# anisanazim/Movie-Recommendation-Engine

Measured on AMD Instinct MI355X. Metric: item embeddings/sec + top-K ANN queries/sec, ML-25M d=256, 1/2/4/8 GPU, higher is better.
Workload: dtype f64 cdf / f32 features / fp4 sign planes (exact integer Hamming); 1 GPU; SYN-25M (ML-25M-shaped: U=162541 M=59047 R=25000095), F=128 H=256 d=256, 2 GCN layers, W=100 L=2 T=10, LSH 512-bit, 10000 queries K=11, rng=numpy (the reference's np.random MT19937 stream generated on device: neighbour ids bit-exact with the reference CPU path); global_items=59047, queries=10000, parallelism=item-shard x1

## Files before the change

### include/pinsage_hip.h

```cpp
#ifndef PINSAGE_HIP_H
#define PINSAGE_HIP_H

#include <stddef.h>
#include <stdint.h>

#ifdef __cplusplus
extern "C" {
#endif

#define PS_OK 0
#define PS_EINVAL (-1)
#define PS_ELAUNCH (-2)
#define PS_EWORKSPACE (-3)
#define PS_EUNSUPPORTED (-4)

#define PS_RNG_STREAM 0
#define PS_RNG_PHILOX 1
#define PS_RNG_STREAM_RAW 2

#define PS_RNG_STREAM_WALKS 3

#define PS_WALK_HALF_BUCKETS 0x100

typedef void *ps_stream_t;
// ... 85 lines not shown
                          ps_stream_t stream);

size_t ps_bn_stats_workspace_bytes(int64_t M, int N);
int ps_bn_batch_stats(const float *z, int64_t M, int N, const float *gamma, float eps, float momentum, float *running_mean,
                      float *running_var, float *mean, float *var, float *scale, void *workspace, size_t workspace_bytes,
                      ps_stream_t stream);
int ps_bn_apply(const float *z, int64_t M, int N, const float *mean, const float *scale, const float *beta, int flags, float *y,
                ps_stream_t stream);

#define PS_RELU 1
#define PS_L2NORM 2
#define PS_WPERM 4
int ps_permute_k(const float *W, int64_t rows, int K, int ld, float *out, ps_stream_t stream);
int ps_linear(const float *x, int64_t M, int K, const float *W, int ldw, const float *b, int N,
              const float *x2, int K2, const float *W2, int ldw2, int flags, float *y, ps_stream_t stream);

size_t ps_gcn_layer_workspace_bytes(int64_t M, int H);
int ps_gcn_layer(const float *x, int64_t M, int K, const float *W, int ldw, const float *b, int N, const float *h_full,
                 int64_t n_full, int H, const int32_t *ids, const int32_t *counts, const float *wts, const int32_t *nvalid,
                 int T, int64_t max_idx, int renorm, const float *W2, int ldw2, int flags, float *y, void *workspace,
                 size_t workspace_bytes, ps_stream_t stream);
int ps_gcn_order(const int32_t *ids, const int32_t *nvalid, int layers, int64_t M, int T, int64_t max_idx, int32_t *ord_out,
                 int32_t *tile_heavy_out, ps_stream_t stream);
int ps_gcn_layer_ordered(const float *x, int64_t M, int K, const float *W, int ldw, const float *b, int N, const float *h_full,
                         int64_t n_full, int H, const int32_t *ids, const int32_t *counts, const float *wts,
                         const int32_t *nvalid, int T, int64_t max_idx, int renorm, const float *W2, int ldw2, int flags, float *y,
                         void *workspace, size_t workspace_bytes, const int32_t *ord, const int32_t *tile_heavy,
                         ps_stream_t stream);

#define PS_LSH_STAGED 8
size_t ps_lsh_stage_bytes(int nbits, int D);
int ps_lsh_stage(const float *A, int nbits, int D, void *staged, size_t staged_bytes, ps_stream_t stream);
int ps_lsh_encode(const float *x, int64_t N, int D, const float *A, int nbits, uint8_t *codes, int flags, ps_stream_t stream);

size_t ps_hamming_topk_workspace_bytes(int64_t nq, int64_t N, int cs, int k);
int ps_hamming_topk(const uint8_t *qcodes, int64_t nq, const uint8_t *codes, int64_t N, int cs, int k,
                    int64_t id_offset, int32_t *dist, int64_t *ids,
                    void *workspace, size_t workspace_bytes, ps_stream_t stream);

size_t ps_lsh_planes_bytes(int64_t n, int cs);
int ps_lsh_expand(const uint8_t *codes, int64_t n, int cs, void *planes, ps_stream_t stream);
size_t ps_hamming_topk_mfma_workspace_bytes(int64_t nq, int64_t N, int cs, int k);
int ps_hamming_topk_mfma(const void *qplanes, int64_t nq, const void *dbplanes, int64_t N, int cs, int k,
                         int64_t id_offset, int32_t *dist, int64_t *ids,
                         void *workspace, size_t workspace_bytes, ps_stream_t stream);
int ps_hamming_topk_mfma_codes(const uint8_t *qcodes, int64_t nq, const void *dbplanes, int64_t N, int cs, int k,
                               int64_t id_offset, int32_t *dist, int64_t *ids,
                               void *workspace, size_t workspace_bytes, ps_stream_t stream);

int ps_topk_merge(const int32_t *dist_in, const int64_t *ids_in, int P, int64_t nq, int k,
                  int32_t *dist, int64_t *ids, ps_stream_t stream);
int ps_topk_merge_strided(const int32_t *dist_in, int64_t dist_stride, const int64_t *ids_in, int64_t ids_stride,
                          int P, int64_t nq, int k, int32_t *dist, int64_t *ids, ps_stream_t stream);

size_t ps_dot_topk_workspace_bytes(int64_t nq, int64_t N, int D, int k);
int ps_dot_topk(const float *E, int64_t N, int D, const int64_t *qidx, int64_t nq, int k, int exclude_self,
                float *vals, int64_t *ids, void *workspace, size_t workspace_bytes, ps_stream_t stream);

int ps_row_dot(const float *A, int64_t nA, const float *B, int64_t nB, int D, const int64_t *ia, const int64_t *ib, int64_t n,
               float *out, ps_stream_t stream);
int ps_rank_count(const float *E, int64_t N, int D, int64_t id_offset, const float *Q, int64_t nq, const float *thr,
                  const int64_t *tid, int64_t *count, ps_stream_t stream);

size_t ps_l2_topk_workspace_bytes(int64_t nq, int64_t N, int D, int k);
int ps_l2_topk(const float *X, int64_t N, int D, const float *Q, int64_t nq, int k, const int32_t *assign,
               const uint32_t *probe, int words, float *dist, int64_t *ids, void *workspace,
// ... 57 lines not shown
```

### movie-recommendation-engine_amd/csrc/hamming_mfma.hip

```cpp
#include "ps_select.h"
#include <type_traits>

namespace {

typedef int v4i __attribute__((ext_vector_type(4)));
typedef int v8i __attribute__((ext_vector_type(8)));
typedef float v16f __attribute__((ext_vector_type(16)));

#ifndef PS_HM_DEBUG
#define PS_HM_DEBUG 0
#endif
#if PS_HM_DEBUG & 32
__device__ unsigned long long ps_hm_counts[8];
#define PS_HM_COUNT(slot, n) do { if (MODE == 1 && lane == 0) atomicAdd(&ps_hm_counts[slot], (unsigned long long)(n)); } while (0)
extern "C" int ps_debug_hm_counts(unsigned long long *host, int reset) {
    unsigned long long z[8] = {};
    if (reset) return (int)hipMemcpyToSymbol(HIP_SYMBOL(ps_hm_counts), z, sizeof(z));
    return (int)hipMemcpyFromSymbol(host, HIP_SYMBOL(ps_hm_counts), sizeof(z));
}
#else
#define PS_HM_COUNT(slot, n) do {} while (0)
#endif
#if PS_HM_DEBUG & 512
__device__ unsigned long long ps_hm_times[4 * 4096];
extern "C" int ps_debug_hm_times_clear() {
    static unsigned long long z[4 * 4096];
    return (int)hipMemcpyToSymbol(HIP_SYMBOL(ps_hm_times), z, sizeof(z));
}
extern "C" int ps_debug_hm_times(unsigned long long *host) {
    return (int)hipMemcpyFromSymbol(host, HIP_SYMBOL(ps_hm_times), sizeof(unsigned long long) * 4 * 4096);
}
#endif
constexpr uint32_t EMPTY_KEY = PS_EMPTY32;
constexpr int NBUF = 4;
constexpr int WAVES = 8;
constexpr int PAD_TILES = 4;
constexpr float NO_DOT = -1048576.0f;
constexpr int entry_tiles(int KS) { return KS >= 4 ? 2 : 4; }
template <int KS> struct EntryTiles { static constexpr int value = entry_tiles(KS); };
template <int KS> struct EntryTiles2 { static constexpr int value = KS >= 8 ? 1 : KS == 4 ? 2 : 4; };
constexpr int ring_entries(bool db) { return db ? NBUF : 3; }
template <int KS, bool DB> constexpr int ring_bytes() {
    return ring_entries(DB) * (DB ? EntryTiles<KS>::value : EntryTiles2<KS>::value) * KS * 1024;
}
constexpr size_t column_bytes(int cap) { return (size_t)WAVES * cap * 64 * sizeof(uint32_t); }

__device__ __forceinline__ uint4 expand_word(uint32_t bits) {
    auto four = [](uint32_t n) { return (n | (n << 3) | (n << 6) | (n << 9)) & 0x1111u; };
    auto eight = [&](uint32_t byte) { return 0xaaaaaaaau ^ ((four(byte & 15u) | (four(byte >> 4) << 16)) << 3); };
    return make_uint4(eight(bits & 255u), eight((bits >> 8) & 255u), eight((bits >> 16) & 255u), eight(bits >> 24));
}

__global__ __launch_bounds__(256) void lsh_expand_kernel(const uint32_t *__restrict__ codes, int64_t n, int KS,
                                                         int64_t pieces, uint4 *__restrict__ planes) {
    for (int64_t p = (int64_t)blockIdx.x * blockDim.x + threadIdx.x; p < pieces; p += (int64_t)gridDim.x * blockDim.x) {
        const int lane = (int)(p & 63);
        const int64_t ts = p >> 6;
        const int s = (int)(ts % KS);
        const int64_t tile = ts / KS;
        const int64_t row = tile * 32 + (lane & 31);
        uint4 o = make_uint4(0u, 0u, 0u, 0u);
        if (row < n) o = expand_word(codes[row * (2 * KS) + 2 * s + (lane >> 5)]);
        planes[p] = o;
    }
}

struct HArgs {
    const unsigned char *qplanes;
    const uint32_t *qcodes;
    const unsigned char *dbplanes;
    int64_t nq, N;
    int64_t tile_begin, tile_end;
    int64_t tiles_per_slice;
    int nqb, slices;
    int k, nbits, shift;
    int cap;
    int64_t id_offset;
    const int32_t *thr0;
    int32_t *bl;
    int list_base;
    int32_t *out_d;
    int32_t *out_r;
};

// ... 946 lines not shown
```

### movie-recommendation-engine_amd/csrc/lsh_filter.hip

```cpp
#include "ps_common.h"

#ifndef PS_LSHF_DEBUG
#define PS_LSHF_DEBUG 0
#endif

#if PS_LSHF_DEBUG
__device__ float *ps_lshf_dump_buf;
extern "C" int ps_debug_lsh_dump(float *buf) { return (int)hipMemcpyToSymbol(HIP_SYMBOL(ps_lshf_dump_buf), &buf, sizeof buf); }
#endif

#if PS_LSHF_DEBUG == 2
#define LSHF_STAMP(slot) do { if (threadIdx.x == 0 && ps_lshf_dump_buf != nullptr) \
    reinterpret_cast<unsigned long long *>(ps_lshf_dump_buf)[(size_t)blockIdx.x * 16 + (slot)] = __builtin_readcyclecounter(); } while (0)
#define LSHF_NOW() __builtin_readcyclecounter()
#define LSHF_PUT(slot, v) do { if (threadIdx.x == 0 && ps_lshf_dump_buf != nullptr) \
    reinterpret_cast<unsigned long long *>(ps_lshf_dump_buf)[(size_t)blockIdx.x * 16 + (slot)] = (v); } while (0)
#else
#define LSHF_STAMP(slot) do {} while (0)
#define LSHF_NOW() 0ull
#define LSHF_PUT(slot, v) do {} while (0)
#endif

namespace {

typedef __bf16 bf16x8 __attribute__((ext_vector_type(8)));
typedef float f32x16 __attribute__((ext_vector_type(16)));
typedef float f32x4 __attribute__((ext_vector_type(4)));

constexpr uint32_t LSHF_MAGIC = 0x4653484cu;
constexpr int HEADER_BYTES = 64;
constexpr int LIST_CAP = 2048;
constexpr int MAX_NBITS = 1024;

// ... 34 lines not shown
#pragma unroll
        for (int e = 0; e < 8; ++e) {
            const float a = row[8 * (e >> 2) + (e & 3)];
            hi[e] = (__bf16)a;
            lo[e] = (__bf16)(a - (float)hi[e]);
        }
        bf16x8 *dst = reinterpret_cast<bf16x8 *>(img + off_slabs + (size_t)jt * slab_f4(KS) * 16);
        dst[(2 * s) * 64 + lane] = hi;
        dst[(2 * s + 1) * 64 + lane] = lo;
    }
    for (int64_t j = t0; j < nbits; j += step) {
        double ss = 0.0;
        for (int k = 0; k < D; ++k) {
            const double a = (double)A[(size_t)j * D + k];
            ss += a * a;
        }
        const double nrm = sqrt(ss);
        float na = __builtin_inff();
        if (nrm >= 0x1p-30 && nrm <= 0x1p30) na = (float)(nrm * (1.0 + 0x1p-10));
        float *dst = reinterpret_cast<float *>(img + off_slabs + ((size_t)(j / 32) * slab_f4(KS) + KS * 128) * 16);
        dst[j % 32] = na;
    }
}

struct FilterArgs {
    const float *x;
    int64_t N;
    const float *a32;
    const f32x4 *slabs;
    int nbits;
    uint32_t *codes;
    unsigned long long *counters;
    float c;
};

template <int KS, int JS>
__global__ __launch_bounds__(256, JS == 1 ? 2 : 1) void lsh_filter_kernel(const FilterArgs g) {
    constexpr int D = KS * 16, ROWS = 128 / JS, RG = 4 / JS, SF4 = slab_f4(KS), NQ = KS / 2;
    extern __shared__ f32x4 lds[];
    __shared__ uint32_t cnt, more;
    const int W = g.nbits / 32;
    f32x4 *slabL = lds;
    uint32_t *codesL = reinterpret_cast<uint32_t *>(lds + JS * SF4);
    uint32_t *flagsL = codesL + W * ROWS;
    uint32_t *listL = flagsL + W * ROWS;

    const int tid = threadIdx.x, lane = tid & 63, wave = tid >> 6;
    const int r = lane & 31, h = lane >> 5;
    const int rg = wave % RG, ph = wave / RG;
    const int64_t row0 = (int64_t)blockIdx.x * ROWS;
    const int64_t row = row0 + rg * 32 + r;
    const bool live = row < g.N;

    LSHF_STAMP(0);
    bf16x8 xh[KS], xl[KS];
    float ss = 0.f;
    {
        const float4 *xr = reinterpret_cast<const float4 *>(g.x + (live ? row : 0) * D);
#pragma unroll
        for (int s = 0; s < KS; ++s) {
#pragma unroll
            for (int t = 0; t < 2; ++t) {
                float4 v = xr[4 * s + 2 * t + h];
                if (!live) v = make_float4(0.f, 0.f, 0.f, 0.f);
                const float e[4] = {v.x, v.y, v.z, v.w};
#pragma unroll
                for (int q = 0; q < 4; ++q) {
                    const __bf16 hi = (__bf16)e[q];
                    xh[s][4 * t + q] = hi;
                    xl[s][4 * t + q] = (__bf16)(e[q] - (float)hi);
                    ss = fmaf(e[q], e[q], ss);
                }
            }
        }
    }
    ss += __shfl_xor(ss, 32);
    float thr = __builtin_inff();
    if (ss >= 0x1p-60f && ss <= 0x1p60f) thr = g.c * (sqrtf(ss) * (1.f + 0x1p-10f));

    const int iters = (W + JS - 1) / JS;
    f32x4 pre[JS][NQ], pna[JS];
#define LSHF_PREFETCH(it_)                                                             \
    _Pragma("unroll") for (int sl = 0; sl < JS; ++sl) {                                \
        const int jt_ = (it_) * JS + sl;                                                \
        if (jt_ < W) {                                                                  \
            const f32x4 *src = g.slabs + (size_t)jt_ * SF4;                            \
            _Pragma("unroll") for (int q = 0; q < NQ; ++q) pre[sl][q] = src[tid + 256 * q]; \
            if (tid < 8) pna[sl] = src[KS * 128 + tid];                                 \
        }                                                                               \
    }
    LSHF_PREFETCH(0)
    LSHF_STAMP(1);
    [[maybe_unused]] unsigned long long t_stage = 0ull, t_mfma = 0ull, t_epi = 0ull;
    for (int it = 0; it < iters; ++it) {
        const unsigned long long c0 = LSHF_NOW();
        __syncthreads();
#pragma unroll
        for (int sl = 0; sl < JS; ++sl) {
            if (it * JS + sl < W) {
#pragma unroll
                for (int q = 0; q < NQ; ++q) slabL[sl * SF4 + tid + 256 * q] = pre[sl][q];
                if (tid < 8) slabL[sl * SF4 + KS * 128 + tid] = pna[sl];
            }
        }
        __syncthreads();
        const unsigned long long c1 = LSHF_NOW();
        t_stage += c1 - c0;
        if (it + 1 < iters) { LSHF_PREFETCH(it + 1) }
        const int jt = it * JS + ph;
        if (jt < W) {
            const f32x4 *sb = slabL + ph * SF4;
            f32x16 acc, acc1;
#pragma unroll
            for (int e = 0; e < 16; ++e) acc[e] = acc1[e] = 0.f;
            f32x4 fh[3], fl[3];
            fh[0] = sb[lane];
            fl[0] = sb[64 + lane];
            if (KS > 1) {
                fh[1] = sb[2 * 64 + lane];
                fl[1] = sb[3 * 64 + lane];
            }
#pragma unroll
            for (int s = 0; s < KS; ++s) {
                if (s + 2 < KS) {
// ... 6 lines not shown
                    acc = __builtin_amdgcn_mfma_f32_32x32x16_bf16(al, xh[s], acc, 0, 0, 0);
                    acc1 = __builtin_amdgcn_mfma_f32_32x32x16_bf16(ah, xl[s], acc1, 0, 0, 0);
                    acc = __builtin_amdgcn_mfma_f32_32x32x16_bf16(ah, xh[s], acc, 0, 0, 0);
                } else {
                    acc1 = __builtin_amdgcn_mfma_f32_32x32x16_bf16(al, xh[s], acc1, 0, 0, 0);
                    acc = __builtin_amdgcn_mfma_f32_32x32x16_bf16(ah, xl[s], acc, 0, 0, 0);
                    acc1 = __builtin_amdgcn_mfma_f32_32x32x16_bf16(ah, xh[s], acc1, 0, 0, 0);
                }
                __builtin_amdgcn_sched_barrier(0);
            }
            acc += acc1;
            const unsigned long long c2 = LSHF_NOW();
            t_mfma += c2 - c1;
            uint32_t sm = 0u, fm = 0u;
#pragma unroll
            for (int gq = 0; gq < 4; ++gq) {
                const f32x4 na = sb[KS * 128 + 2 * gq + h];
#pragma unroll
                for (int q = 0; q < 4; ++q) {
                    const float f = acc[4 * gq + q];
#if PS_LSHF_DEBUG == 1
                    if (ps_lshf_dump_buf != nullptr && live) ps_lshf_dump_buf[row * g.nbits + jt * 32 + 8 * gq + 4 * h + q] = f;
#endif
                    const bool trusted = __builtin_fabsf(f) > thr * na[q];
                    sm |= (trusted && f >= 0.f ? 1u : 0u) << (8 * gq + q);
                    fm |= (trusted ? 0u : 1u) << (8 * gq + q);
                }
            }
            sm <<= 4 * h;
            fm <<= 4 * h;
            if (!live) fm = 0u;
            sm |= (uint32_t)__shfl_xor((int)sm, 32);
            fm |= (uint32_t)__shfl_xor((int)fm, 32);
            if (h == 0) {
                codesL[jt * ROWS + rg * 32 + r] = sm;
                flagsL[jt * ROWS + rg * 32 + r] = fm;
            }
            t_epi += LSHF_NOW() - c2;
        }
    }

#undef LSHF_PREFETCH
    LSHF_STAMP(2);
    LSHF_PUT(6, t_stage);
    LSHF_PUT(7, t_mfma);
    LSHF_PUT(8, t_epi);

    const int nwords = W * ROWS;
    unsigned long long nflag = 0ull;
    for (;;) {
        __syncthreads();
        if (tid == 0) {
            cnt = 0u;
            more = 0u;
        }
        __syncthreads();
        int mine = 0;
#pragma unroll 4
        for (int idx = tid; idx < nwords; idx += 256) mine += __builtin_popcount(flagsL[idx]);
        if (mine > 0) {
            uint32_t pos = atomicAdd(&cnt, (uint32_t)mine);
            if (pos + (uint32_t)mine > (uint32_t)LIST_CAP) more = 1u;
            for (int idx = tid; idx < nwords && pos < (uint32_t)LIST_CAP; idx += 256) {
                uint32_t m = flagsL[idx];
                if (m == 0u) continue;
                while (m != 0u && pos < (uint32_t)LIST_CAP) {
                    listL[pos++] = (uint32_t)idx * 32u + (uint32_t)__builtin_ctz(m);
                    m &= m - 1u;
                }
                flagsL[idx] = m;
            }
        }
        __syncthreads();
        LSHF_STAMP(3);
        const int n = cnt < (uint32_t)LIST_CAP ? (int)cnt : LIST_CAP;
        const bool again = more != 0u;
        for (int e = tid; e < n; e += 256) {
            const uint32_t ent = listL[e];
            const int idx = (int)(ent >> 5), b = (int)(ent & 31u);
            const int jt = idx / ROWS, rl = idx % ROWS;
            const float4 *xr = reinterpret_cast<const float4 *>(g.x + (row0 + rl) * D);
            const float4 *ar = reinterpret_cast<const float4 *>(g.a32 + (size_t)(jt * 32 + b) * D);
            float acc = 0.f;
#pragma unroll 16
            for (int k = 0; k < D / 4; ++k) {
                const float4 u = xr[k], v = ar[k];
                acc = fmaf(u.x, v.x, acc);
                acc = fmaf(u.y, v.y, acc);
                acc = fmaf(u.z, v.z, acc);
                acc = fmaf(u.w, v.w, acc);
            }
            if (acc >= 0.f) atomicOr(&codesL[idx], 1u << b);
        }
        nflag += (unsigned long long)n;
        if (!again) break;
    }
    __syncthreads();
    LSHF_STAMP(4);

    for (int i = tid; i < nwords; i += 256) {
        const int rl = i / W, w = i % W;
        if (row0 + rl < g.N) g.codes[(row0 + rl) * W + w] = codesL[w * ROWS + rl];
    }
    if (g.counters != nullptr && tid == 0) {
        const int64_t rows = g.N - row0 < ROWS ? g.N - row0 : ROWS;
        atomicAdd(g.counters, (unsigned long long)rows * (unsigned long long)g.nbits);
        atomicAdd(g.counters + 1, nflag);
    }
    LSHF_STAMP(5);
}

template <int KS, int JS>
size_t filter_lds(int nbits) {
    return (size_t)JS * slab_f4(KS) * 16 + (size_t)(nbits / 32) * (128 / JS) * 8 + (size_t)LIST_CAP * 4;
}

template <int KS, int JS>
int launch_filter(const FilterArgs &g, hipStream_t st) {
    const int64_t grid = ps_cdiv(g.N, 128 / JS);
    if (grid > 0x7fffffff) return PS_EUNSUPPORTED;
    const size_t lds = filter_lds<KS, JS>(g.nbits);
    hipLaunchKernelGGL((lsh_filter_kernel<KS, JS>), dim3((unsigned)grid), dim3(256), lds, st, g);
    PS_CHECK_LAUNCH();
    return PS_OK;
}

template <int KS, int JS>
bool allow_lds() {
    return ps_allow_lds(lsh_filter_kernel<KS, JS>, filter_lds<KS, JS>(MAX_NBITS));
}

}

extern "C" size_t ps_lsh_stage_bytes(int nbits, int D) { return served(nbits, D) ? stage_layout(nbits, D).total : 0; }

extern "C" int ps_lsh_stage(const float *A, int nbits, int D, void *staged, size_t staged_bytes, ps_stream_t stream) {
    if (nbits <= 0 || D <= 0 || !A || !staged) return PS_EINVAL;
    if (!served(nbits, D) || (reinterpret_cast<size_t>(A) | reinterpret_cast<size_t>(staged)) % 16 != 0) return PS_EUNSUPPORTED;
    const StageLayout l = stage_layout(nbits, D);
    if (staged_bytes < l.total) return PS_EINVAL;
    int64_t grid = ps_cdiv((int64_t)nbits * D, 256);
    if (grid > 1024) grid = 1024;
    hipLaunchKernelGGL(lsh_stage_kernel, dim3((unsigned)grid), dim3(256), 0, ps_stream(stream), A, nbits, D,
                       static_cast<unsigned char *>(staged), l.a32, l.slabs);
    PS_CHECK_LAUNCH();
    return PS_OK;
}

int psi_lsh_encode_staged(const float *x, int64_t N, int D, const void *staged, int nbits, uint8_t *codes, ps_stream_t stream) {
    if (!served(nbits, D) || (reinterpret_cast<size_t>(x) | reinterpret_cast<size_t>(staged)) % 16 != 0) return PS_EUNSUPPORTED;
    static PsPerDevice cus;
    int dv = 0;
    if (!ps_device_index(&dv)) return PS_ELAUNCH;
    int ncu = cus.get(dv);
    if (ncu == 0) {
        if (!(allow_lds<2, 1>() && allow_lds<4, 1>() && allow_lds<8, 1>() && allow_lds<16, 1>() && allow_lds<2, 2>() &&
              allow_lds<4, 2>() && allow_lds<8, 2>() && allow_lds<16, 2>()))
            return PS_ELAUNCH;
        if (hipDeviceGetAttribute(&ncu, hipDeviceAttributeMultiprocessorCount, dv) != hipSuccess || ncu <= 0) return PS_ELAUNCH;
        cus.set(dv, ncu);
    }
    const StageLayout l = stage_layout(nbits, D);
    const unsigned char *img = static_cast<const unsigned char *>(staged);
    const char *se = getenv("PS_LSH_STATS"), *re = getenv("PS_LSH_ROWS");
    FilterArgs g;
    g.x = x;
    g.N = N;
    g.a32 = reinterpret_cast<const float *>(img + l.a32);
    g.slabs = reinterpret_cast<const f32x4 *>(img + l.slabs);
    g.nbits = nbits;
    g.codes = reinterpret_cast<uint32_t *>(codes);
    g.counters = se && atoi(se) != 0 ? reinterpret_cast<unsigned long long *>(const_cast<unsigned char *>(img) + 16) : nullptr;
    g.c = 0x1p-12f * (D > 256 ? (float)D / 256.f : 1.f);
    const int rows = re ? atoi(re) : 0;
    const bool half = rows == 64 || (rows != 128 && ps_cdiv(N, 128) * 2 <= ncu);
    hipStream_t st = ps_stream(stream);
    switch (D / 16) {
        case 2: return half ? launch_filter<2, 2>(g, st) : launch_filter<2, 1>(g, st);
        case 4: return half ? launch_filter<4, 2>(g, st) : launch_filter<4, 1>(g, st);
        case 8: return half ? launch_filter<8, 2>(g, st) : launch_filter<8, 1>(g, st);
        default: return half ? launch_filter<16, 2>(g, st) : launch_filter<16, 1>(g, st);
    }
}
```

### movie-recommendation-engine_amd/pinsage_hip/dense.py

```python
from __future__ import annotations

import os

import torch

from . import native as nv


def _rowmajor(w):
    if w.dtype != torch.float32:
        raise TypeError("fp32 expected")
    if w.dim() != 2:
        raise ValueError("2-D matrix expected")
    if w.stride(1) != 1 or w.stride(0) < w.size(1):
        w = w.contiguous()
    return w, w.stride(0) if w.size(0) > 1 else max(w.stride(0), w.size(1))


def _require_cuda(*tensors):
    for t in tensors:
        if t is not None and not t.is_cuda:
            raise nv.NativeError("libpinsage_hip takes device (HBM) tensors; got a CPU tensor (no CPU fallback)")


# ... 186 lines not shown
    if max_idx is None:
        max_idx = n_full - 1
    if b is not None:
        b = b.contiguous()
    ids, nvalid = ids.contiguous(), nvalid.contiguous()
    counts = counts.contiguous() if counts is not None else None
    wts = wts.contiguous() if wts is not None else None
    flags = (nv.PS_RELU if relu else 0) | (nv.PS_L2NORM if l2norm else 0) | (nv.PS_WPERM if staged else 0)
    ws, wsb = nv.workspace("ps_gcn_layer_workspace_bytes", x.device, M, H)
    if wsb > 0:
        y = torch.empty((M, N), dtype=torch.float32, device=x.device)
        if order is not None:
            ord_, heavy = order
            if ord_.dtype != torch.int32 or heavy.dtype != torch.int32 or ord_.numel() != (M + 63) // 64 * 64 \
                    or heavy.numel() != (M + 63) // 64:
                raise ValueError("order: (int32[64 * ceil(M / 64)], int32[ceil(M / 64)]) of gcn_orders expected")
        with torch.cuda.device(x.device):
            if order is not None:
                rc = nv.lib().ps_gcn_layer_ordered(nv.ptr(x), M, K, nv.ptr(Wk, contiguous=False), ldw, nv.ptr(b), N, nv.ptr(h_full),
                                                   n_full, H, nv.ptr(ids), nv.ptr(counts), nv.ptr(wts), nv.ptr(nvalid), T, int(max_idx),
                                                   int(renorm), nv.ptr(W2k, contiguous=False), ldw2, flags, nv.ptr(y), nv.ptr(ws), wsb,
                                                   nv.ptr(ord_), nv.ptr(heavy), nv.stream())
            else:
                rc = nv.lib().ps_gcn_layer(nv.ptr(x), M, K, nv.ptr(Wk, contiguous=False), ldw, nv.ptr(b), N, nv.ptr(h_full), n_full, H,
                                           nv.ptr(ids), nv.ptr(counts), nv.ptr(wts), nv.ptr(nvalid), T, int(max_idx), int(renorm),
                                           nv.ptr(W2k, contiguous=False), ldw2, flags, nv.ptr(y), nv.ptr(ws), wsb, nv.stream())
        if rc != nv.PS_EUNSUPPORTED:
            nv.check(rc, "ps_gcn_layer")
            return y
    h_neigh = sampling.importance_pool(h_full, ids=ids, counts=counts, wts=wts, nvalid=nvalid, max_idx=max_idx, renorm=renorm)
    return linear(x, W, b, x2=h_neigh, W2=W2, relu=relu, l2norm=l2norm)


def lsh_encode(x, A):
    flags = nv.PS_LSH_STAGED if isinstance(A, StagedLsh) else nv.PS_WPERM if isinstance(A, StagedWeight) else 0
    if flags == nv.PS_LSH_STAGED:
        nbits, da, A = A.shape[0], A.shape[1], A.image
    elif flags:
        A = A.t
    _require_cuda(x, A)
    x = x.contiguous()
    A = A.contiguous()
    n, d = x.size(0), x.size(1)
    if flags != nv.PS_LSH_STAGED:
        nbits, da = A.size(0), A.size(1)
    if da != d:
        raise ValueError("projection matrix must be [nbits, dim]")
    codes = torch.empty((n, nbits // 8), dtype=torch.uint8, device=x.device)
    with torch.cuda.device(x.device):
        nv.call("ps_lsh_encode", nv.ptr(x), n, d, nv.ptr(A), nbits, nv.ptr(codes), flags, nv.stream())
    return codes


HAMMING_MAX_K = 64


def lsh_expand(codes):
    _require_cuda(codes)
    codes = codes.contiguous()
    n, cs = codes.size(0), codes.size(1)
    planes, nb = nv.workspace("ps_lsh_planes_bytes", codes.device, n, cs)
    if nb:
        with torch.cuda.device(codes.device):
            nv.call("ps_lsh_expand", nv.ptr(codes), n, cs, nv.ptr(planes), nv.stream())
    return planes


def hamming_mfma_supported(nq, N, cs, k):
    return nv.lib().ps_hamming_topk_mfma_workspace_bytes(nq, N, cs, k) > 0


def hamming_topk(qcodes, codes, k, id_offset=0, planes=None, use_mfma=True, out=None):
    _require_cuda(qcodes, codes)
    qcodes = qcodes.contiguous()
    codes = codes.contiguous()
    nq, cs = qcodes.size(0), qcodes.size(1)
    N = codes.size(0)
    if out is not None:
        dist, ids = out
        if (tuple(dist.shape) != (nq, k) or tuple(ids.shape) != (nq, k) or dist.dtype != torch.int32
                or ids.dtype != torch.int64 or not dist.is_contiguous() or not ids.is_contiguous()):
            raise ValueError("out must be contiguous (int32 [nq, k], int64 [nq, k])")
    if k > HAMMING_MAX_K or cs > 128 or (cs & (cs - 1)) != 0 or cs % 4 != 0:
        d, i = _hamming_topk_large_k(qcodes, codes, k, id_offset)
# ... 292 lines not shown
```

### movie-recommendation-engine_amd/pinsage_hip/native.py

```python
from __future__ import annotations

import ctypes as C
import os

import torch

_HERE = os.path.dirname(os.path.abspath(__file__))
SO_PATH = os.environ.get("PS_HIP_LIB") or os.path.join(_HERE, "libpinsage_hip.so")
_lib = None

PS_RNG_STREAM = 0
PS_RNG_PHILOX = 1
PS_RNG_STREAM_RAW = 2
PS_RNG_STREAM_WALKS = 3
PS_WALK_HALF_BUCKETS = 0x100
PS_RELU = 1
PS_L2NORM = 2
PS_WPERM = 4
PS_LSH_STAGED = 8
PS_HN_PER_QUERY, PS_HN_EXCLUDE_DIAG = 1, 2
PS_LOSS_SHARED, PS_LOSS_PER_QUERY, PS_LOSS_BATCH_HARD = 0, 1, 2
PS_PPR_NO_SKIP = 1
PS_OK, PS_EINVAL, PS_ELAUNCH, PS_EWORKSPACE, PS_EUNSUPPORTED = 0, -1, -2, -3, -4

# ... 22 lines not shown
    "ps_graph_stats": "i ppqqpp",
    "ps_walk_sample": "i pppqpqiiiippQIppppppppp",
    "ps_walk_sample_layers": "i pppqpqiiiippqQIpppppipppp",
    "ps_walk_paths": "i pppqpqiippQIipppp",
    "ps_uniform_offsets": "i pqpqiippp",
    "ps_mt19937_chunk_log2": "i",
    "ps_mt19937_window_shift": "i",
    "ps_mt19937_raw_stream": "i piqppppipipipipzp",
    "ps_mt19937_workspace_bytes": "z qq",
    "ps_mt19937_random_sample": "i piqqppppipipipzp",
    "ps_importance_pool": "i pqippppqiqipp",
    "ps_attention_weights": "i ppqipppqipp",
    "ps_gather_max": "i pqippqipp",
    "ps_pool_weights": "i ppppqiqiipp",
    "ps_gather_bwd_segment": "i",
    "ps_gather_bwd_workspace_bytes": "z qii",
    "ps_gather_bwd": "i ppqipppqippzp",
    "ps_gather_max_arg": "i pqippqippp",
    "ps_attention_bwd_rows_workspace_bytes": "z qi",
    "ps_attention_bwd_rows": "i pqippipppppqippppzp",
    "ps_attention_bwd_cols": "i ppqipppipqppzp",
    "ps_bn_stats_workspace_bytes": "z qi",
    "ps_bn_batch_stats": "i pqipffppppppzp",
    "ps_bn_apply": "i pqipppipp",
    "ps_permute_k": "i pqiipp",
    "ps_linear": "i pqipipipipiipp",
    "ps_gcn_layer_workspace_bytes": "z qi",
    "ps_gcn_layer": "i pqipipipqippppiqipiippzp",
    "ps_gcn_order": "i ppiqiqppp",
    "ps_gcn_layer_ordered": "i pqipipipqippppiqipiippzppp",
    "ps_lsh_stage_bytes": "z ii",
    "ps_lsh_stage": "i piipzp",
    "ps_lsh_encode": "i pqipipip",
    "ps_hamming_topk_workspace_bytes": "z qqii",
    "ps_hamming_topk": "i pqpqiiqpppzp",
    "ps_lsh_planes_bytes": "z qi",
    "ps_lsh_expand": "i pqipp",
    "ps_hamming_topk_mfma_workspace_bytes": "z qqii",
    "ps_hamming_topk_mfma": "i pqpqiiqpppzp",
    "ps_hamming_topk_mfma_codes": "i pqpqiiqpppzp",
    "ps_topk_merge": "i ppiqippp",
    "ps_topk_merge_strided": "i pqpqiqippp",
    "ps_dot_topk_workspace_bytes": "z qqii",
    "ps_dot_topk": "i pqipqiipppzp",
    "ps_row_dot": "i pqpqippqpp",
    "ps_rank_count": "i pqiqpqpppp",
    "ps_l2_topk_workspace_bytes": "z qqii",
    "ps_l2_topk": "i pqipqippipppzp",
    "ps_ivf_topk_workspace_bytes": "z qqiiiiq",
    "ps_ivf_topk": "i pqipiqppqpiipppzp",
    "ps_spmm_csr": "i ppppqiqqpp",
    "ps_cooc_planes_bytes": "z qqi",
    "ps_cooc_planes": "i pppqqqipzppp",
    "ps_cooc_pairs": "i pqqiqpqpqppp",
    "ps_cooc_pairs_sparse_workspace_bytes": "z qi",
    "ps_cooc_pairs_sparse": "i pppppppqqqqqipqpppzp",
    "ps_cooc_keys": "i pqqqppppppqpp",
    "ps_cooc_emit": "i ppqppp",
    "ps_hardest_negative": "i pqipqipppp",
    "ps_margin_loss": "i ppqipfppppp",
    "ps_margin_loss_bwd": "i pppqqiippppppp",
    "ps_ppr_shares": "i ppqpp",
    "ps_ppr_push_workspace_bytes": "z qq",
    "ps_ppr_push": "i pppqqppipqQiippzp",
    "ps_ppr_topk": "i pqqqqippppp",
}
# ... 23 lines not shown
    return _lib


def check(rc: int, what: str):
    if rc != 0:
        raise NativeError(f"{what}: {lib().ps_error_string(rc).decode()} (code {rc})")


class KernelTimer:

    def __init__(self):
        self.events = []

    def summary(self):
        torch.cuda.synchronize()
        out = {}
        for name, a, b in self.events:
            d = out.setdefault(name, {"launches": 0, "ms": 0.0})
            d["launches"] += 1
            d["ms"] += a.elapsed_time(b)
        for d in out.values():
            d["avg_ms"] = d["ms"] / d["launches"]
        return out


_timer = None


def set_timer(t):
    global _timer
    _timer = t


def call(name, *args):
    fn = getattr(lib(), name)
    if _timer is None:
        rc = fn(*args)
    else:
        a, b = torch.cuda.Event(enable_timing=True), torch.cuda.Event(enable_timing=True)
        a.record()
        rc = fn(*args)
        b.record()
        _timer.events.append((name, a, b))
    check(rc, name)


def ptr(t, contiguous=True):
    if t is None:
        return C.c_void_p(0)
    if not t.is_cuda:
        raise NativeError("libpinsage_hip takes device (HBM) pointers; got a CPU tensor")
    if contiguous and not t.is_contiguous():
        raise NativeError("tensor must be contiguous")
    return C.c_void_p(t.data_ptr())


def workspace(bytes_fn, device, *dims):
    nbytes = getattr(lib(), bytes_fn)(*dims)
    return (torch.empty(nbytes, dtype=torch.uint8, device=device) if nbytes else None), nbytes


_raw_stream = getattr(torch._C, "_cuda_getCurrentRawStream", None)
_get_device = getattr(torch._C, "_cuda_getDevice", None)


def stream():
    if _raw_stream is not None and _get_device is not None:
        return C.c_void_p(_raw_stream(_get_device()))
    return C.c_void_p(torch.cuda.current_stream().cuda_stream)


def require_gpu():
    if not torch.cuda.is_available():
        raise NativeError("the PinSage hot path needs an MI355X (torch.cuda is not available); "
                          "there is no CPU fallback")
    lib()
    return torch.device("cuda", torch.cuda.current_device())
# ... 7 lines not shown
```

### movie-recommendation-engine_amd/pinsage_hip/shard.py

```python
from __future__ import annotations

import os

import torch
import torch.distributed as dist

from . import dense, sampling


def shard_range(M, rank, world):
    chunk = (M + world - 1) // world
    lo = min(rank * chunk, M)
    return lo, min(lo + chunk, M), chunk


def _backend(group):
    return dist.get_backend(group) if dist.is_initialized() else None


class _Gather:

    def __init__(self, out, work=None, dev=None):
        self.out, self.work, self.dev = out, work, dev

# ... 72 lines not shown

class HipOps:

    def sample(self, sampler, nodes, T, shard=None):
        if shard is not None and getattr(sampler, "rng", None) == "numpy":
            M, lo = shard
            all_nodes = torch.arange(M, dtype=torch.int64, device=nodes.device)
            return sampler.sample_batch(nodes, T, stream_nodes=(all_nodes, lo))
        return sampler.sample_batch(nodes, T)

    def sample_layers(self, sampler, lo, hi, T, layers, shard=None):
        stream = None
        if shard is not None and getattr(sampler, "rng", None) == "numpy":
            stream = (range(shard[0]), shard[1])
        return sampler.sample_batches(range(lo, hi), T, layers, stream_nodes=stream, defer_state=True)

    def finish(self):
        dense.finish_rng_state()

    def pool(self, h_full, batch, max_idx):
        return sampling.importance_pool(h_full, batch, max_idx=max_idx)

    def linear(self, x, W, b, x2=None, W2=None, relu=False, l2norm=False):
        return dense.linear(x, W, b, x2=x2, W2=W2, relu=relu, l2norm=l2norm)

    def gcn_layer(self, x, W, b, h_full, batch, max_idx, W2, order=None):
        return dense.gcn_layer(x, W, b, h_full, batch.ids, batch.counts, batch.nvalid, W2, max_idx=max_idx, order=order)

    def gcn_orders(self, batches, max_idx):
        return dense.gcn_orders([b.ids for b in batches], [b.nvalid for b in batches], max_idx)

    def lsh_encode(self, x, A):
        return dense.lsh_encode(x, A)

    def stage_weight(self, W):
        return dense.stage_weight(W)

    def stage_lsh(self, A):
        return dense.stage_lsh(A)

    def lsh_planes(self, codes):
        return dense.lsh_expand(codes)

    def hamming_topk(self, q, codes, k, id_offset, planes=None, out=None):
        return dense.hamming_topk(q, codes, k, id_offset=id_offset, planes=planes, out=out)

    def topk_merge(self, d, i):
        return dense.topk_merge(d, i)

    def topk_merge_records(self, records, nq, k):
        return dense.topk_merge_records(records, nq, k)


class ShardedPinSage:

    def __init__(self, params, num_layers, sampler, num_items, ops=None, group=None, standin=None):
        self.P = params
        self.num_layers = num_layers
        self.sampler = sampler
        self.M = int(num_items)
        self.ops = ops if ops is not None else HipOps()
        self.group = group
        self.comm = Comm(group, standin=standin)
        self.rank, self.world = self.comm.rank, self.comm.world
        self.lo, self.hi, self.chunk = shard_range(self.M, self.rank, self.world)
        self._nodes = {}
# ... 98 lines not shown
            Wu = P[f"convs.{i}.lin_update.weight"]
            if self.fuse_self:
                W1, b1 = self._fused_layer(i, H)
                a_in = h
            else:
                a_in = ops.linear(h, P[f"convs.{i}.lin_self.weight"], P[f"convs.{i}.lin_self.bias"])
                W1, b1 = Wu[:, :H], P[f"convs.{i}.lin_update.bias"]
            h_full = pending.wait()
            if side is not None:
                torch.cuda.current_stream(dev).wait_event(ready[i])
            if self.fuse_self and hasattr(ops, "gcn_layer"):
                kw = {} if orders is None else {"order": orders[i]}
                h = ops.gcn_layer(a_in, self._w(("l1", i), W1), b1, h_full, batches[i], self.M - 1, self._w(("l2", i), Wu[:, H:]), **kw)
            else:
                h_neigh = ops.pool(h_full, batches[i], self.M - 1)
                h = ops.linear(a_in, self._w(("l1", i), W1), b1, x2=h_neigh, W2=self._w(("l2", i), Wu[:, H:]), relu=True, l2norm=True)
            if i + 1 < self.num_layers:
                pending = self.comm.gather_rows_async(h, self.chunk, "h")
        return ops.linear(h, self._w("out", P["output_proj.weight"]), P["output_proj.bias"], l2norm=True)

    def _staged_A(self, A):
        stage = getattr(self.ops, "stage_lsh", None) or getattr(self.ops, "stage_weight", None)
        if stage is None or not isinstance(A, torch.Tensor):
            return A
        ent = self._staged.get("A")
        if ent is None or ent[0] is not A or ent[1] != A._version:
            ent = self._staged["A"] = (A, A._version, stage(A))
        return ent[2]

    REPLICATE_CODES_BYTES = 64 << 20

    def build_index(self, emb_local, A):
        self.A = A
        self.codes = self.ops.lsh_encode(emb_local, self._staged_A(A))
        self.codes_all = None
        if self.world > 1 and self.M * int(self.codes.size(1)) <= self.REPLICATE_CODES_BYTES:
            self.codes_all = self.comm.gather_rows(self.codes, self.chunk, "codes")[: self.M]
        scanned = self.codes_all if self.codes_all is not None else self.codes
        self.planes = self.ops.lsh_planes(scanned) if hasattr(self.ops, "lsh_planes") else None
        return self.codes

    def search(self, q_local, k):
        ops = self.ops
        qc = ops.lsh_encode(q_local, self._staged_A(self.A))
        nq_local = qc.size(0)
        planes = getattr(self, "planes", None)
        if self.world > 1 and getattr(self, "codes_all", None) is not None:
            n = nq_local * k
            rec = (12 * n + 15) // 16 * 16
            mine = self.comm._buf("res", "mine", (1, rec), torch.uint8, qc.device, zero=True)
            ids_v = mine[0, : 8 * n].view(torch.int64).view(nq_local, k)
            dist_v = mine[0, 8 * n: 12 * n].view(torch.int32).view(nq_local, k)
            try:
                ops.hamming_topk(qc, self.codes_all, k, 0, planes=planes, out=(dist_v, ids_v))
            except TypeError:
                d, i = ops.hamming_topk(qc, self.codes_all, k, 0)
                dist_v.copy_(d)
                ids_v.copy_(i)
            allr = self.comm.gather_rows(mine, 1, "res")
            P_ = self.world
            return (allr[:, 8 * n: 12 * n].view(torch.int32).reshape(P_ * nq_local, k),
                    allr[:, : 8 * n].view(torch.int64).reshape(P_ * nq_local, k))
        qc_all = self.comm.gather_rows(qc, nq_local, "qcodes")
        if self.world == 1:
            return (ops.hamming_topk(qc_all, self.codes, k, self.lo, planes=planes) if planes is not None
                    else ops.hamming_topk(qc_all, self.codes, k, self.lo))
# ... 19 lines not shown
```

### movie-recommendation-engine_amd/utils/nearest_neighbors.py

```python
from __future__ import annotations

import time

import numpy as np
import torch

from pinsage_hip import dense
from pinsage_hip import native as nv

_INT_MAX_F = np.float32(2147483647)


def _faiss_float_randn(n, seed):
    def raw_stream(sd):
        bg = np.random.MT19937()
        bg._legacy_seeding(int(sd) & 0xFFFFFFFF)
        return bg
    g0 = raw_stream(seed)
    a0, b0 = (int(v) & 0x7FFFFFFF for v in g0.random_raw(2))
    nblock = 1 if n < 1024 else 1024
    out = np.empty(n, dtype=np.float32)
    inv = 1.0 / 4294967295.0
    for j in range(nblock):
        lo, hi = j * n // nblock, (j + 1) * n // nblock
# ... 64 lines not shown
        self.planes = None
        self.use_mfma = True
        self.device = nv.require_gpu()
        if self.rotate_data:
            A = lsh_rotation_matrix(self.d, self.nbits, seed=5, recipe=recipe)
        else:
            if self.d < self.nbits:
                raise ValueError("d >= nbits is required without rotate_data")
            A = np.eye(self.nbits, self.d, dtype=np.float32)
        self._set_A(A)

    def _set_A(self, A):
        A = torch.as_tensor(A, dtype=torch.float32)
        words = 1
        while words * 32 < A.size(0) and words < 32:
            words *= 2
        if words * 32 < A.size(0):
            words = (int(A.size(0)) + 31) // 32
        pad = words * 32 - A.size(0)
        if pad:
            A = torch.cat([A, torch.zeros((pad, A.size(1)), dtype=torch.float32)], dim=0)
        self.A = A.to(self.device).contiguous()
        self._staged = None

    def _staged_A(self):
        ent = self._staged
        if ent is None or ent[0] is not self.A or ent[1] != self.A._version:
            ent = self._staged = (self.A, self.A._version, dense.stage_lsh(self.A))
        return ent[2]

    def train(self, x):
        return None

    def _encode(self, x):
        x = torch.as_tensor(x, dtype=torch.float32).to(self.device)
        if x.dim() != 2 or x.size(1) != self.d:
            raise AssertionError(f"expected [n, {self.d}] vectors")
        return dense.lsh_encode(x, self._staged_A())

    def add(self, x):
        c = self._encode(x)
        self.codes = c if self.codes is None else torch.cat([self.codes, c], dim=0)
        self.ntotal = int(self.codes.size(0))
        self.planes = dense.lsh_expand(self.codes) if int(self.codes.size(1)) in (8, 16, 32, 64) else None

    def reset(self):
        self.codes, self.planes, self.ntotal = None, None, 0

    def search_device(self, x, k, id_offset=0):
        q = self._encode(x)
        codes = self.codes if self.codes is not None else torch.empty((0, self.code_size), dtype=torch.uint8,
                                                                       device=self.device)
        return dense.hamming_topk(q, codes, int(k), id_offset=id_offset, planes=self.planes, use_mfma=self.use_mfma)

    def search(self, x, k):
        dist, ids = self.search_device(x, k)
        d = dist.cpu().numpy().astype(np.float32)
        i = ids.cpu().numpy()
        d[i < 0] = _INT_MAX_F
        return d, i


class LSHIndex:

    rotation_recipe = "numpy"

    def __init__(self, dim, num_bits=256, num_tables=16):
        self.dim = dim
        self.num_bits = num_bits
        self.num_tables = num_tables
        self.index = _DeviceLSH(dim, num_bits, num_tables, recipe=self.rotation_recipe)

    def set_rotation(self, A):
        A = torch.as_tensor(A, dtype=torch.float32)
        if tuple(A.shape) != (self.num_bits, self.dim):
            raise ValueError("rotation must be [num_bits, dim]")
        self.index._set_A(A)
# ... 238 lines not shown
```

Measured before the change: 47.52 million items/s.

## Fuse LSH plane expansion into filter kernel and restructure flagged-bit refinement

The LSH filter kernel now writes the expanded fp4 sign planes directly from its LDS codes, so the separate lsh_expand pass is skipped when building the index. The flagged-word list is also built during the MFMA loop through per-wave segments, which removes the first full popcount scan. For JS==1 the exact dot-product refinement becomes a cooperative LDS-staged, prefetched computation in place of one thread per entry streaming rows. The cost is more LDS, more register pressure and extra complexity, plus a fallback path that expands separately when the fused path is unsupported.

```diff
diff --git a/include/pinsage_hip.h b/include/pinsage_hip.h
--- a/include/pinsage_hip.h
+++ b/include/pinsage_hip.h
@@ -141,6 +141,8 @@
 size_t ps_lsh_stage_bytes(int nbits, int D);
 int ps_lsh_stage(const float *A, int nbits, int D, void *staged, size_t staged_bytes, ps_stream_t stream);
 int ps_lsh_encode(const float *x, int64_t N, int D, const float *A, int nbits, uint8_t *codes, int flags, ps_stream_t stream);
+int ps_lsh_encode_planes(const float *x, int64_t N, int D, const void *staged, int nbits, uint8_t *codes, void *planes,
+                         ps_stream_t stream);
 
 size_t ps_hamming_topk_workspace_bytes(int64_t nq, int64_t N, int cs, int k);
 int ps_hamming_topk(const uint8_t *qcodes, int64_t nq, const uint8_t *codes, int64_t N, int cs, int k,
diff --git a/movie-recommendation-engine_amd/csrc/hamming_mfma.hip b/movie-recommendation-engine_amd/csrc/hamming_mfma.hip
--- a/movie-recommendation-engine_amd/csrc/hamming_mfma.hip
+++ b/movie-recommendation-engine_amd/csrc/hamming_mfma.hip
@@ -1,4 +1,5 @@
 #include "ps_select.h"
+#include "lsh_planes.h"
 #include <type_traits>
 
 namespace {
@@ -44,12 +45,6 @@
     return ring_entries(DB) * (DB ? EntryTiles<KS>::value : EntryTiles2<KS>::value) * KS * 1024;
 }
 constexpr size_t column_bytes(int cap) { return (size_t)WAVES * cap * 64 * sizeof(uint32_t); }
-
-__device__ __forceinline__ uint4 expand_word(uint32_t bits) {
-    auto four = [](uint32_t n) { return (n | (n << 3) | (n << 6) | (n << 9)) & 0x1111u; };
-    auto eight = [&](uint32_t byte) { return 0xaaaaaaaau ^ ((four(byte & 15u) | (four(byte >> 4) << 16)) << 3); };
-    return make_uint4(eight(bits & 255u), eight((bits >> 8) & 255u), eight((bits >> 16) & 255u), eight(bits >> 24));
-}
 
 __global__ __launch_bounds__(256) void lsh_expand_kernel(const uint32_t *__restrict__ codes, int64_t n, int KS,
                                                          int64_t pieces, uint4 *__restrict__ planes) {
diff --git a/movie-recommendation-engine_amd/csrc/lsh_filter.hip b/movie-recommendation-engine_amd/csrc/lsh_filter.hip
--- a/movie-recommendation-engine_amd/csrc/lsh_filter.hip
+++ b/movie-recommendation-engine_amd/csrc/lsh_filter.hip
@@ -1,4 +1,5 @@
 #include "ps_common.h"
+#include "lsh_planes.h"
 
 #ifndef PS_LSHF_DEBUG
 #define PS_LSHF_DEBUG 0
@@ -99,18 +100,27 @@
     uint32_t *codes;
     unsigned long long *counters;
     float c;
+    uint4 *planes;
+    int64_t plane_pieces;
 };
+
+__host__ __device__ constexpr int area_f4(int KS, int JS) {
+    return JS == 1 && slab_f4(KS) < 2048 ? 2048 : JS * slab_f4(KS);
+}
 
 template <int KS, int JS>
 __global__ __launch_bounds__(256, JS == 1 ? 2 : 1) void lsh_filter_kernel(const FilterArgs g) {
     constexpr int D = KS * 16, ROWS = 128 / JS, RG = 4 / JS, SF4 = slab_f4(KS), NQ = KS / 2;
+    constexpr int PF = KS >= 16 ? 4 : 2;
     extern __shared__ f32x4 lds[];
-    __shared__ uint32_t cnt, more;
+    constexpr int SEG = LIST_CAP / 4;
+    __shared__ uint32_t cnt, more, segn[4];
     const int W = g.nbits / 32;
     f32x4 *slabL = lds;
-    uint32_t *codesL = reinterpret_cast<uint32_t *>(lds + JS * SF4);
+    uint32_t *codesL = reinterpret_cast<uint32_t *>(lds + area_f4(KS, JS));
     uint32_t *flagsL = codesL + W * ROWS;
     uint32_t *listL = flagsL + W * ROWS;
+    uint16_t *wordL = reinterpret_cast<uint16_t *>(listL + LIST_CAP);
 
     const int tid = threadIdx.x, lane = tid & 63, wave = tid >> 6;
     const int r = lane & 31, h = lane >> 5;
@@ -157,6 +167,11 @@
         }                                                                               \
     }
     LSHF_PREFETCH(0)
+    if (tid == 0) {
+        cnt = 0u;
+        more = 0u;
+    }
+    int wcnt = 0;
     LSHF_STAMP(1);
     [[maybe_unused]] unsigned long long t_stage = 0ull, t_mfma = 0ull, t_epi = 0ull;
     for (int it = 0; it < iters; ++it) {
@@ -229,6 +244,14 @@
             if (!live) fm = 0u;
             sm |= (uint32_t)__shfl_xor((int)sm, 32);
             fm |= (uint32_t)__shfl_xor((int)fm, 32);
+            const bool fw = h == 0 && fm != 0u;
+            const unsigned long long wm = __ballot(fw);
+            if (fw) {
+                const int at = wcnt + (int)__builtin_amdgcn_mbcnt_lo((uint32_t)wm, 0u);
+                if (at < SEG) wordL[wave * SEG + at] = (uint16_t)(jt * ROWS + rg * 32 + r);
+                else more = 1u;
+            }
+            wcnt += __builtin_popcountll(wm);
             if (h == 0) {
                 codesL[jt * ROWS + rg * 32 + r] = sm;
                 flagsL[jt * ROWS + rg * 32 + r] = fm;
@@ -238,26 +261,125 @@
     }
 
 #undef LSHF_PREFETCH
+    if (lane == 0) segn[wave] = (uint32_t)(wcnt < SEG ? wcnt : SEG);
     LSHF_STAMP(2);
     LSHF_PUT(6, t_stage);
     LSHF_PUT(7, t_mfma);
     LSHF_PUT(8, t_epi);
 
     const int nwords = W * ROWS;
+    const f32x4 *xb = reinterpret_cast<const f32x4 *>(g.x + row0 * D), *ab = reinterpret_cast<const f32x4 *>(g.a32);
+    f32x4 *pieceL = lds;
     unsigned long long nflag = 0ull;
+    __syncthreads();
+    const int s1 = (int)segn[0], s2 = s1 + (int)segn[1], s3 = s2 + (int)segn[2];
+    const int nw = s3 + (int)segn[3];
+    for (int e = tid; e < nw; e += 256) {
+        const int w = (e >= s1 ? 1 : 0) + (e >= s2 ? 1 : 0) + (e >= s3 ? 1 : 0);
+        const uint32_t idx = wordL[w * SEG + e - (w == 3 ? s3 : w == 2 ? s2 : w == 1 ? s1 : 0)];
+        uint32_t m = flagsL[idx];
+        listL[e] = idx * 32u + (uint32_t)__builtin_ctz(m);
+        m &= m - 1u;
+        if (m != 0u) {
+            uint32_t pos = (uint32_t)nw + atomicAdd(&cnt, (uint32_t)__builtin_popcount(m));
+            while (m != 0u && pos < (uint32_t)LIST_CAP) {
+                listL[pos++] = idx * 32u + (uint32_t)__builtin_ctz(m);
+                m &= m - 1u;
+            }
+            if (m != 0u) more = 1u;
+        }
+        flagsL[idx] = m;
+    }
+    __syncthreads();
+    int n = (uint32_t)nw + cnt < (uint32_t)LIST_CAP ? nw + (int)cnt : LIST_CAP;
+    bool again = more != 0u;
+    LSHF_STAMP(3);
     for (;;) {
+        if constexpr (JS == 2) {
+            for (int e = tid; e < n; e += 256) {
+                const uint32_t ent = listL[e];
+                const int idx = (int)(ent >> 5), b = (int)(ent & 31u);
+                const f32x4 *xr = xb + (idx % ROWS) * (D / 4), *ar = ab + ((idx / ROWS) * 32 + b) * (D / 4);
+                float acc = 0.f;
+#pragma unroll 16
+                for (int k = 0; k < D / 4; ++k) {
+                    const f32x4 u = xr[k], v = ar[k];
+                    acc = fmaf(u[0], v[0], acc);
+                    acc = fmaf(u[1], v[1], acc);
+                    acc = fmaf(u[2], v[2], acc);
+                    acc = fmaf(u[3], v[3], acc);
+                }
+                if (acc >= 0.f) atomicOr(&codesL[idx], 1u << b);
+            }
+        }
+        for (int base = 0; JS == 1 && base < n; base += 256) {
+            const int m = n - base < 256 ? n - base : 256;
+            const int q = tid & 3, sw = (tid >> 4) & 3;
+            int xo[4], ao[4];
+#pragma unroll
+            for (int i = 0; i < 4; ++i) {
+                const int el = 64 * i + (tid >> 2);
+                const uint32_t ent = listL[base + (el < m ? el : 0)];
+                const int idx = (int)(ent >> 5), b = (int)(ent & 31u);
+                xo[i] = (idx % ROWS) * (D / 4) + q;
+                ao[i] = ((idx / ROWS) * 32 + b) * (D / 4) + q;
+            }
+            const uint32_t mine = listL[base + (tid < m ? tid : 0)];
+            f32x4 px[PF][4], pa[PF][4];
+#pragma unroll
+            for (int p = 0; p < PF; ++p) {
+#pragma unroll
+                for (int i = 0; i < 4; ++i) {
+                    px[p][i] = xb[xo[i] + 4 * p];
+                    pa[p][i] = ab[ao[i] + 4 * p];
+                }
+            }
+            float acc = 0.f;
+#pragma unroll
+            for (int p = 0; p < KS; ++p) {
+                __syncthreads();
+#pragma unroll
+                for (int i = 0; i < 4; ++i) {
+                    const int at = (64 * i + (tid >> 2)) * 4 + (q ^ sw);
+                    pieceL[at] = px[p % PF][i];
+                    pieceL[1024 + at] = pa[p % PF][i];
+                }
+                __syncthreads();
+                if (p + PF < KS) {
+#pragma unroll
+                    for (int i = 0; i < 4; ++i) {
+                        px[p % PF][i] = xb[xo[i] + 4 * (p + PF)];
+                        pa[p % PF][i] = ab[ao[i] + 4 * (p + PF)];
+                    }
+                }
+                if (tid < m) {
+                    const int so = (tid >> 2) & 3;
+#pragma unroll
+                    for (int j = 0; j < 4; ++j) {
+                        const f32x4 u = pieceL[tid * 4 + (j ^ so)], v = pieceL[1024 + tid * 4 + (j ^ so)];
+                        acc = fmaf(u[0], v[0], acc);
+                        acc = fmaf(u[1], v[1], acc);
+                        acc = fmaf(u[2], v[2], acc);
+                        acc = fmaf(u[3], v[3], acc);
+                    }
+                }
+            }
+            if (tid < m && acc >= 0.f) atomicOr(&codesL[mine >> 5], 1u << (mine & 31u));
+        }
+        nflag += (unsigned long long)n;
+        if (!again) break;
         __syncthreads();
         if (tid == 0) {
             cnt = 0u;
             more = 0u;
         }
         __syncthreads();
-        int mine = 0;
+        int own = 0;
 #pragma unroll 4
-        for (int idx = tid; idx < nwords; idx += 256) mine += __builtin_popcount(flagsL[idx]);
-        if (mine > 0) {
-            uint32_t pos = atomicAdd(&cnt, (uint32_t)mine);
-            if (pos + (uint32_t)mine > (uint32_t)LIST_CAP) more = 1u;
+        for (int idx = tid; idx < nwords; idx += 256) own += __builtin_popcount(flagsL[idx]);
+        if (own > 0) {
+            uint32_t pos = atomicAdd(&cnt, (uint32_t)own);
+            if (pos + (uint32_t)own > (uint32_t)LIST_CAP) more = 1u;
             for (int idx = tid; idx < nwords && pos < (uint32_t)LIST_CAP; idx += 256) {
                 uint32_t m = flagsL[idx];
                 if (m == 0u) continue;
@@ -269,28 +391,8 @@
             }
         }
         __syncthreads();
-        LSHF_STAMP(3);
-        const int n = cnt < (uint32_t)LIST_CAP ? (int)cnt : LIST_CAP;
-        const bool again = more != 0u;
-        for (int e = tid; e < n; e += 256) {
-            const uint32_t ent = listL[e];
-            const int idx = (int)(ent >> 5), b = (int)(ent & 31u);
-            const int jt = idx / ROWS, rl = idx % ROWS;
-            const float4 *xr = reinterpret_cast<const float4 *>(g.x + (row0 + rl) * D);
-            const float4 *ar = reinterpret_cast<const float4 *>(g.a32 + (size_t)(jt * 32 + b) * D);
-            float acc = 0.f;
-#pragma unroll 16
-            for (int k = 0; k < D / 4; ++k) {
-                const float4 u = xr[k], v = ar[k];
-                acc = fmaf(u.x, v.x, acc);
-                acc = fmaf(u.y, v.y, acc);
-                acc = fmaf(u.z, v.z, acc);
-                acc = fmaf(u.w, v.w, acc);
-            }
-            if (acc >= 0.f) atomicOr(&codesL[idx], 1u << b);
-        }
-        nflag += (unsigned long long)n;
-        if (!again) break;
+        n = cnt < (uint32_t)LIST_CAP ? (int)cnt : LIST_CAP;
+        again = more != 0u;
     }
     __syncthreads();
     LSHF_STAMP(4);
@@ -298,6 +400,19 @@
     for (int i = tid; i < nwords; i += 256) {
         const int rl = i / W, w = i % W;
         if (row0 + rl < g.N) g.codes[(row0 + rl) * W + w] = codesL[w * ROWS + rl];
+    }
+    if (g.planes != nullptr) {
+        const int KP = W / 2;
+        const int64_t first = (int64_t)blockIdx.x * (ROWS / 32) * KP * 64;
+        for (int i = tid; i < nwords; i += 256) {
+            const int ln = i & 63, ts = i >> 6;
+            const int rl = (ts / KP) * 32 + (ln & 31), w = 2 * (ts % KP) + (ln >> 5);
+            uint4 o = make_uint4(0u, 0u, 0u, 0u);
+            if (row0 + rl < g.N) o = expand_word(codesL[w * ROWS + rl]);
+            if (first + i < g.plane_pieces) g.planes[first + i] = o;
+        }
+        if (blockIdx.x == gridDim.x - 1)
+            for (int64_t i = first + nwords + tid; i < g.plane_pieces; i += 256) g.planes[i] = make_uint4(0u, 0u, 0u, 0u);
     }
     if (g.counters != nullptr && tid == 0) {
         const int64_t rows = g.N - row0 < ROWS ? g.N - row0 : ROWS;
@@ -309,7 +424,7 @@
 
 template <int KS, int JS>
 size_t filter_lds(int nbits) {
-    return (size_t)JS * slab_f4(KS) * 16 + (size_t)(nbits / 32) * (128 / JS) * 8 + (size_t)LIST_CAP * 4;
+    return (size_t)area_f4(KS, JS) * 16 + (size_t)(nbits / 32) * (128 / JS) * 8 + (size_t)LIST_CAP * 4 + (size_t)LIST_CAP * 2;
 }
 
 template <int KS, int JS>
@@ -344,7 +459,8 @@
     return PS_OK;
 }
 
-int psi_lsh_encode_staged(const float *x, int64_t N, int D, const void *staged, int nbits, uint8_t *codes, ps_stream_t stream) {
+static int encode_staged(const float *x, int64_t N, int D, const void *staged, int nbits, uint8_t *codes, void *planes,
+                         size_t planes_bytes, ps_stream_t stream) {
     if (!served(nbits, D) || (reinterpret_cast<size_t>(x) | reinterpret_cast<size_t>(staged)) % 16 != 0) return PS_EUNSUPPORTED;
     static PsPerDevice cus;
     int dv = 0;
@@ -369,6 +485,8 @@
     g.codes = reinterpret_cast<uint32_t *>(codes);
     g.counters = se && atoi(se) != 0 ? reinterpret_cast<unsigned long long *>(const_cast<unsigned char *>(img) + 16) : nullptr;
     g.c = 0x1p-12f * (D > 256 ? (float)D / 256.f : 1.f);
+    g.planes = static_cast<uint4 *>(planes);
+    g.plane_pieces = (int64_t)(planes_bytes / 16);
     const int rows = re ? atoi(re) : 0;
     const bool half = rows == 64 || (rows != 128 && ps_cdiv(N, 128) * 2 <= ncu);
     hipStream_t st = ps_stream(stream);
@@ -379,3 +497,16 @@
         default: return half ? launch_filter<16, 2>(g, st) : launch_filter<16, 1>(g, st);
     }
 }
+
+int psi_lsh_encode_staged(const float *x, int64_t N, int D, const void *staged, int nbits, uint8_t *codes, ps_stream_t stream) {
+    return encode_staged(x, N, D, staged, nbits, codes, nullptr, 0, stream);
+}
+
+extern "C" int ps_lsh_encode_planes(const float *x, int64_t N, int D, const void *staged, int nbits, uint8_t *codes, void *planes,
+                                    ps_stream_t stream) {
+    if (N < 0 || D <= 0 || nbits <= 0 || !x || !staged || !codes || !planes) return PS_EINVAL;
+    const size_t planes_bytes = ps_lsh_planes_bytes(N, nbits / 8);
+    if (planes_bytes == 0 || nbits % 64 != 0 || !served(nbits, D)) return PS_EUNSUPPORTED;
+    if (reinterpret_cast<size_t>(codes) % 4 != 0 || reinterpret_cast<size_t>(planes) % 16 != 0) return PS_EUNSUPPORTED;
+    return encode_staged(x, N, D, staged, nbits, codes, planes, planes_bytes, stream);
+}
diff --git a/movie-recommendation-engine_amd/csrc/lsh_planes.h b/movie-recommendation-engine_amd/csrc/lsh_planes.h
--- /dev/null
+++ b/movie-recommendation-engine_amd/csrc/lsh_planes.h
@@ -0,0 +1,9 @@
+#pragma once
+#include <hip/hip_runtime.h>
+#include <stdint.h>
+
+__device__ __forceinline__ uint4 expand_word(uint32_t bits) {
+    auto four = [](uint32_t n) { return (n | (n << 3) | (n << 6) | (n << 9)) & 0x1111u; };
+    auto eight = [&](uint32_t byte) { return 0xaaaaaaaau ^ ((four(byte & 15u) | (four(byte >> 4) << 16)) << 3); };
+    return make_uint4(eight(bits & 255u), eight((bits >> 8) & 255u), eight((bits >> 16) & 255u), eight(bits >> 24));
+}
diff --git a/movie-recommendation-engine_amd/pinsage_hip/dense.py b/movie-recommendation-engine_amd/pinsage_hip/dense.py
--- a/movie-recommendation-engine_amd/pinsage_hip/dense.py
+++ b/movie-recommendation-engine_amd/pinsage_hip/dense.py
@@ -242,7 +242,7 @@
     return linear(x, W, b, x2=h_neigh, W2=W2, relu=relu, l2norm=l2norm)
 
 
-def lsh_encode(x, A):
+def lsh_encode(x, A, planes=False):
     flags = nv.PS_LSH_STAGED if isinstance(A, StagedLsh) else nv.PS_WPERM if isinstance(A, StagedWeight) else 0
     if flags == nv.PS_LSH_STAGED:
         nbits, da, A = A.shape[0], A.shape[1], A.image
@@ -257,9 +257,17 @@
     if da != d:
         raise ValueError("projection matrix must be [nbits, dim]")
     codes = torch.empty((n, nbits // 8), dtype=torch.uint8, device=x.device)
+    if planes and flags == nv.PS_LSH_STAGED:
+        pl, nb = nv.workspace("ps_lsh_planes_bytes", x.device, n, nbits // 8)
+        if nb:
+            with torch.cuda.device(x.device):
+                rc = nv.call("ps_lsh_encode_planes", nv.ptr(x), n, d, nv.ptr(A), nbits, nv.ptr(codes), nv.ptr(pl), nv.stream(),
+                             unsupported_ok=True)
+            if rc == nv.PS_OK:
+                return codes, pl
     with torch.cuda.device(x.device):
         nv.call("ps_lsh_encode", nv.ptr(x), n, d, nv.ptr(A), nbits, nv.ptr(codes), flags, nv.stream())
-    return codes
+    return (codes, lsh_expand(codes)) if planes else codes
 
 
 HAMMING_MAX_K = 64
diff --git a/movie-recommendation-engine_amd/pinsage_hip/native.py b/movie-recommendation-engine_amd/pinsage_hip/native.py
--- a/movie-recommendation-engine_amd/pinsage_hip/native.py
+++ b/movie-recommendation-engine_amd/pinsage_hip/native.py
@@ -78,6 +78,7 @@
     "ps_lsh_stage_bytes": "z ii",
     "ps_lsh_stage": "i piipzp",
     "ps_lsh_encode": "i pqipipip",
+    "ps_lsh_encode_planes": "i pqipippp",
     "ps_hamming_topk_workspace_bytes": "z qqii",
     "ps_hamming_topk": "i pqpqiiqpppzp",
     "ps_lsh_planes_bytes": "z qi",
@@ -167,7 +168,10 @@
     _timer = t
 
 
-def call(name, *args):
+_TIMER_NAMES = {"ps_lsh_encode_planes": "ps_lsh_encode"}
+
+
+def call(name, *args, unsupported_ok=False):
     fn = getattr(lib(), name)
     if _timer is None:
         rc = fn(*args)
@@ -176,8 +180,11 @@
         a.record()
         rc = fn(*args)
         b.record()
-        _timer.events.append((name, a, b))
+        _timer.events.append((_TIMER_NAMES.get(name, name), a, b))
+    if unsupported_ok and rc == PS_EUNSUPPORTED:
+        return rc
     check(rc, name)
+    return rc
 
 
 def ptr(t, contiguous=True):
diff --git a/movie-recommendation-engine_amd/pinsage_hip/shard.py b/movie-recommendation-engine_amd/pinsage_hip/shard.py
--- a/movie-recommendation-engine_amd/pinsage_hip/shard.py
+++ b/movie-recommendation-engine_amd/pinsage_hip/shard.py
@@ -128,6 +128,9 @@
 
     def lsh_encode(self, x, A):
         return dense.lsh_encode(x, A)
+
+    def lsh_encode_planes(self, x, A):
+        return dense.lsh_encode(x, A, planes=True)
 
     def stage_weight(self, W):
         return dense.stage_weight(W)
@@ -292,6 +295,11 @@
 
     def build_index(self, emb_local, A):
         self.A = A
+        if hasattr(self.ops, "lsh_encode_planes") and (self.world == 1
+                                                       or self.M * (int(A.shape[0]) // 8) > self.REPLICATE_CODES_BYTES):
+            self.codes, self.planes = self.ops.lsh_encode_planes(emb_local, self._staged_A(A))
+            self.codes_all = None
+            return self.codes
         self.codes = self.ops.lsh_encode(emb_local, self._staged_A(A))
         self.codes_all = None
         if self.world > 1 and self.M * int(self.codes.size(1)) <= self.REPLICATE_CODES_BYTES:
diff --git a/movie-recommendation-engine_amd/utils/nearest_neighbors.py b/movie-recommendation-engine_amd/utils/nearest_neighbors.py
--- a/movie-recommendation-engine_amd/utils/nearest_neighbors.py
+++ b/movie-recommendation-engine_amd/utils/nearest_neighbors.py
@@ -120,17 +120,20 @@
     def train(self, x):
         return None
 
-    def _encode(self, x):
+    def _encode(self, x, planes=False):
         x = torch.as_tensor(x, dtype=torch.float32).to(self.device)
         if x.dim() != 2 or x.size(1) != self.d:
             raise AssertionError(f"expected [n, {self.d}] vectors")
-        return dense.lsh_encode(x, self._staged_A())
+        return dense.lsh_encode(x, self._staged_A(), planes=planes)
 
     def add(self, x):
-        c = self._encode(x)
-        self.codes = c if self.codes is None else torch.cat([self.codes, c], dim=0)
+        with_planes = int(self.A.size(0)) // 8 in (8, 16, 32, 64)
+        if self.codes is None and with_planes:
+            self.codes, self.planes = self._encode(x, planes=True)
+        else:
+            self.codes = torch.cat([self.codes, self._encode(x)], dim=0) if self.codes is not None else self._encode(x)
+            self.planes = dense.lsh_expand(self.codes) if with_planes else None
         self.ntotal = int(self.codes.size(0))
-        self.planes = dense.lsh_expand(self.codes) if int(self.codes.size(1)) in (8, 16, 32, 64) else None
 
     def reset(self):
         self.codes, self.planes, self.ntotal = None, None, 0
```

Result: faster. 48.09 million items/s, median of 6 (+1.2%).
